# google-research/Splat-SLAM

Measured on AMD Instinct MI355X. Metric: mapping frames/sec + render ms @640x480, 300k Gaussians; PSNR vs ref, higher is better.
Workload: dtype f32

## Files before the change

splat_slam_amd/csrc/sgr_api.hip:

```cpp
#include <cstdarg>
#include <cstdio>
#include <cstring>
#include <cstdlib>
#include <vector>

#include <hip/hip_runtime.h>

#include "sgr_common.h"

namespace sgr {

void launch_preprocess_fwd(const ViewTab&, int, const LOff&, const Common&, const SgrInputs&, hipStream_t);
void launch_preprocess_bwd(const ViewTab&, int, const LOff&, const Common&, const SgrInputs&, const SgrGradInputs&, const FusedAdam*,
                           hipStream_t, bool mapping_loop = false);
void launch_binning(const ViewTab&, int, const LOff&, hipStream_t);
void launch_zero_heads(const ViewTab&, int, const LOff&, size_t, hipStream_t);
void launch_blend_fwd(const ViewTab&, int, const LOff&, const float*, const LossTab*, const LossCoef*, hipStream_t);
void launch_blend_bwd(const ViewTab&, int, const LOff&, const float*, const LossTab*, const LossCoef*, hipStream_t);
void launch_blend_fused(const ViewTab&, int, const LOff&, const float*, const LossTab&, const LossCoef&, hipStream_t);
bool blend_can_fuse(const LOff&);

static int g_opt[SGR_OPT_COUNT] = {1, 0, 0};

static thread_local char g_err[512] = "";
int set_error(int code, const char* fmt, ...) {
  va_list ap;
  va_start(ap, fmt);
  vsnprintf(g_err, sizeof(g_err), fmt, ap);
  va_end(ap);
  return code;
}
#define HIP_TRY(expr)                                                                                   \
  do {                                                                                                  \
    hipError_t _e = (expr);                                                                             \
    if (_e != hipSuccess) return set_error(SGR_ERR_HIP, "%s failed: %s", #expr, hipGetErrorString(_e)); \
  } while (0)
// ... 267 lines not shown
      LOff d = L.dev();
      launch_blend_bwd(tab, 1, d, m.settings.bg, nullptr, nullptr, st);
      launch_preprocess_bwd(tab, 1, d, cm, *in, gv, nullptr, st);
    }
    HIP_TRY(hipGetLastError());
    return SGR_OK;
  }
  Layout L = make_layout(f.settings.num_gaussians, f.settings.image_height, f.settings.image_width, f.ws.capacity);
  LOff d = L.dev();
  Common cm = make_common(&f.settings);
  for (int base = 0; base < num_views; base += kMaxViews) {
    const int nv = num_views - base < kMaxViews ? num_views - base : kMaxViews;
    ViewTab tab = {};
    for (int v = 0; v < nv; ++v) {
      const SgrBackwardView& m = views[base + v];
      if (int rc = check_workspace(&m.ws, L)) return rc;
      tab_set_view(tab, v, &m.settings, nullptr, &m.ws);
      tab.radii[v] = const_cast<int32_t*>(m.radii);
      tab.dL_dcolor[v] = m.dL_dcolor; tab.dL_ddepth[v] = m.dL_ddepth; tab.dL_dtau[v] = m.dL_dtau; tab.dL_dmeans2D[v] = m.dL_dmeans2D;
    }
    SgrGradInputs gv = g;
    gv.accumulate = (grad_in->accumulate || base > 0) ? 1 : 0;
    launch_blend_bwd(tab, nv, d, f.settings.bg, nullptr, nullptr, st);
    launch_preprocess_bwd(tab, nv, d, cm, *in, gv, nullptr, st);
  }
  HIP_TRY(hipGetLastError());
  return SGR_OK;
}

}

static int map_views_impl(int32_t num_views, const SgrMapView* views, const SgrInputs* in, const SgrGradInputs* grads, float alpha,
                          float rgb_boundary_threshold, int32_t forward_only, FusedAdam* fused, bool* fused_done,
                          void* stream, bool store_sinks = false, const SgrSsimTerm* term = nullptr) {
  if (fused_done) *fused_done = false;
  if (num_views < 0 || (num_views > 0 && (!views || !in)) || (!forward_only && !grads))
    return set_error(SGR_ERR_INVALID, "map_views: null argument");
  if (num_views == 0) return SGR_OK;
  if (forward_only) term = nullptr;
  if (term) {
    if (!term->arena || term->max_views <= 0)
      return set_error(SGR_ERR_INVALID, "map_views: SSIM term without an arena");
    for (int v = 0; v < num_views; ++v) {
      const SgrMapView& m = views[v];
      const int H = m.settings.image_height, W = m.settings.image_width;
      if (!m.out.color || !m.out.depth || !m.out.opacity)
        return set_error(SGR_ERR_INVALID, "map_views: the SSIM loss needs every view's rendered image, depth and opacity");
      if (term->arena_bytes < sgr_ssim_term_bytes(term->max_views, H, W))
        return set_error(SGR_ERR_WORKSPACE, "map_views: SSIM arena too small (need %zu for %d views of %dx%d)",
                         sgr_ssim_term_bytes(term->max_views, H, W), term->max_views, W, H);
      if (!m.loss_scratch || m.loss_scratch_bytes < (size_t)ssim_loss_nparts(H, W) * sizeof(LossPart))
        return set_error(SGR_ERR_WORKSPACE, "map_views: loss_scratch too small for the SSIM loss (need %zu)",
                         (size_t)ssim_loss_nparts(H, W) * sizeof(LossPart));
    }
  }
  hipStream_t st = (hipStream_t)stream;
  bool uniform = true;
  const SgrMapView& f = views[0];
  for (int v = 0; v < num_views; ++v) {
    const SgrMapView& m = views[v];
    if (int rc = check_settings(&m.settings, in)) return rc;
    uniform = uniform && m.settings.num_gaussians == f.settings.num_gaussians && m.settings.image_height == f.settings.image_height &&
              m.settings.image_width == f.settings.image_width && m.settings.tanfovx == f.settings.tanfovx &&
              m.settings.tanfovy == f.settings.tanfovy && m.settings.scale_modifier == f.settings.scale_modifier &&
              m.settings.sh_degree == f.settings.sh_degree && m.settings.sh_coeffs == f.settings.sh_coeffs &&
              m.settings.bg == f.settings.bg &&
              m.ws.capacity == f.ws.capacity;
// ... 38 lines not shown
  }
  Layout L = make_layout(f.settings.num_gaussians, f.settings.image_height, f.settings.image_width, f.ws.capacity);
  LOff d = L.dev();
  int hint = 0;
  for (int v = 0; v < num_views; ++v) hint = views[v].ws.max_list_hint > hint ? views[v].ws.max_list_hint : hint;
  d.set_hint(hint);
  Common cm = make_common(&f.settings);
  const int HW = f.settings.image_height * f.settings.image_width;
  for (int base = 0; base < num_views; base += kMaxViews) {
    const int nv = num_views - base < kMaxViews ? num_views - base : kMaxViews;
    ViewTab tab = {};
    LossTab lt = {};
    bool all_clean = true;
    for (int v = 0; v < nv; ++v) {
      const SgrMapView& m = views[base + v];
      all_clean = all_clean && m.ws.counters_clean != 0;
      if (int rc = check_workspace(&m.ws, L)) return rc;
      const bool no_images = !m.out.color && !m.out.depth && !m.out.opacity && !forward_only;
      if ((!no_images && (!m.out.color || !m.out.depth || !m.out.opacity)) || !m.out.radii)
        return set_error(SGR_ERR_INVALID, "map_views: null output pointer");
      tab_set_view(tab, v, &m.settings, &m.out, &m.ws);
      if (!forward_only) {
        if (!m.gt_image || !m.gt_depth || !m.dL_dimage || !m.dL_ddepth || !m.loss_scratch ||
            m.loss_scratch_bytes < (size_t)L.ntiles * sizeof(LossPart))
          return set_error(SGR_ERR_INVALID, "map_views: loss buffers missing (loss_scratch needs 16 B per 8x8 tile = %zu)",
                           (size_t)L.ntiles * sizeof(LossPart));
        tab.dL_dcolor[v] = m.dL_dimage; tab.dL_ddepth[v] = m.dL_ddepth; tab.dL_dtau[v] = m.dL_dtau;
        lt.image[v] = m.out.color; lt.depth[v] = m.out.depth; lt.gt_image[v] = m.gt_image; lt.gt_depth[v] = m.gt_depth;
        lt.exp_a[v] = m.exposure_a; lt.exp_b[v] = m.exposure_b; lt.loss[v] = m.loss; lt.dimage[v] = m.dL_dimage;
        lt.ddepth[v] = m.dL_ddepth; lt.da[v] = m.dL_dexposure; lt.db[v] = m.dL_dexposure ? m.dL_dexposure + 1 : nullptr;
        lt.parts[v] = m.loss_scratch;
      }
    }
    if (int rc = forward_batch(tab, nv, L, cm, *in, st, all_clean, d.mean_hint)) return rc;
    if (forward_only) {
      launch_blend_fwd(tab, nv, d, f.settings.bg, nullptr, nullptr, st);
      continue;
    }
    LossCoef lc = {alpha / (3.f * (float)HW), (1.f - alpha) / (float)HW, rgb_boundary_threshold};
    const bool fused_blend = !term && g_opt[SGR_OPT_FUSED_BLEND] != 0 && blend_can_fuse(d);
    int nparts = L.ntiles;
    if (term) {
      const int H = f.settings.image_height, W = f.settings.image_width;
      launch_blend_fwd(tab, nv, d, f.settings.bg, nullptr, nullptr, st);
      for (int g0 = 0; g0 < nv; g0 += term->max_views)
        launch_ssim_mapping_loss(lt, g0, nv - g0 < term->max_views ? nv - g0 : term->max_views, H, W, alpha, term->lambda_dssim,
                                 rgb_boundary_threshold, 1.f, (float*)term->arena, st);
      nparts = ssim_loss_nparts(H, W);
    } else if (fused_blend) {
      launch_blend_fused(tab, nv, d, f.settings.bg, lt, lc, st);
    } else {
      launch_blend_fwd(tab, nv, d, f.settings.bg, &lt, &lc, st);
    }
    const bool fuse = fused && num_views <= kMaxViews;
    if (fuse) {
      fused->tail_views = nv; fused->tail_nparts = nparts;
      fused->tail_inv_rgb = 1.f / (3.f * (float)HW); fused->tail_inv_dep = 1.f / (float)HW; fused->tail_alpha = alpha;
      for (int v = 0; v < nv; ++v) {
        fused->tail_parts[v] = lt.parts[v]; fused->tail_loss[v] = lt.loss[v]; fused->tail_da[v] = lt.da[v]; fused->tail_db[v] = lt.db[v];
      }
    } else {
      launch_mapping_loss_final(lt, nv, HW, nparts, alpha, st);
    }
    if (term) launch_blend_bwd(tab, nv, d, f.settings.bg, nullptr, nullptr, st);
    else if (!fused_blend) launch_blend_bwd(tab, nv, d, f.settings.bg, &lt, &lc, st);
    launch_preprocess_bwd(tab, nv, d, cm, *in, *grads, fuse ? fused : nullptr, st, true);
    if (fuse && fused_done) *fused_done = true;
  }
  HIP_TRY(hipGetLastError());
  return SGR_OK;
}

extern "C" {

int sgr_map_views(int32_t num_views, const SgrMapView* views, const SgrInputs* in, const SgrGradInputs* grads, float alpha,
                  float rgb_boundary_threshold, int32_t forward_only, void* stream) {
  return map_views_impl(num_views, views, in, grads, alpha, rgb_boundary_threshold, forward_only, nullptr, nullptr, stream);
}

}

static int map_step_impl(const SgrMapStep* p, bool skip_activate, bool grads_clean, bool allow_fuse, bool* fused_out, void* stream,
                         const SgrSsimTerm* term = nullptr) {
  if (fused_out) *fused_out = false;
  if (!p) return set_error(SGR_ERR_INVALID, "map_step: null argument");
  const bool adam_only = p->num_views == 0 && p->adam_groups;
  if (!skip_activate && !adam_only && (p->scaling || p->rotation || p->opacity))
    if (int rc = sgr_activate(p->num_gaussians, p->scaling, p->rotation, p->opacity, p->scales_out, p->rot_out, p->opac_out, stream)) return rc;
  FusedAdam fa;
  bool try_fuse = false;
  if (allow_fuse && p->adam_groups && p->num_views > 0 && p->num_views <= kMaxViews && !p->forward_only && p->grads && p->in && p->views) {
    const SgrGradInputs& g = *p->grads;
    const SgrAdamGroup* G = p->adam_groups;
    try_fuse = g.accumulate && g.dL_dmeans3D == G[0].grad && g.dL_dshs == G[1].grad && g.dL_dopacities == G[2].grad &&
               g.dL_dscales == G[3].grad && g.dL_drotations == G[4].grad && !g.dL_dmeans2D && !g.dL_dcolors_precomp &&
               !g.dL_dcov3D_precomp && p->in->shs && !p->in->colors_precomp && p->in->scales && p->in->rotations &&
               p->num_gaussians == p->views[0].settings.num_gaussians;
    for (int v = 0; v < p->num_views && try_fuse; ++v)
      try_fuse = !p->views[v].dL_dtau && p->views[v].settings.sh_degree == 0 && p->views[v].settings.sh_coeffs == 1;
    if (try_fuse) {
      if (int rc = make_fused_adam(p->num_gaussians, G, p->beta1, p->beta2, p->eps, p->iso_weight, &fa)) return rc;
      fa.grads_clean = grads_clean ? 1 : 0;
      fa.s_out = p->scales_out; fa.r_out = p->rot_out; fa.o_out = p->opac_out;
      fa.stat_accum = g.stat_grad_accum;
      fa.stat_denom = g.stat_grad_accum ? g.stat_denom : nullptr;
      fa.stat_maxr = g.stat_grad_accum ? g.stat_max_radii : nullptr;
      if (p->exp_rows > 0) {
        if (!p->exp_param || !p->exp_grad || !p->exp_avg || !p->exp_avg_sq || !p->exp_step || !p->exp_active || p->exp_row_width <= 0)
          return set_error(SGR_ERR_INVALID, "map_step: exposure block incomplete");
        fa.exp_rows = p->exp_rows; fa.exp_width = p->exp_row_width; fa.exp_param = p->exp_param; fa.exp_grad = p->exp_grad;
        fa.exp_avg = p->exp_avg; fa.exp_avg_sq = p->exp_avg_sq; fa.exp_step = p->exp_step; fa.exp_active = p->exp_active;
        fa.exp_lr = p->exp_lr; fa.exp_b1 = p->exp_beta1; fa.exp_b2 = p->exp_beta2; fa.exp_eps = p->exp_eps;
      }
    }
  }
  if ((p->grads_clean == -2 || p->grads_clean == -3) && !p->adam_groups && p->num_views > 0 && p->num_views <= kMaxViews && !p->forward_only && p->grads &&
      p->in && p->views) {
    const SgrGradInputs& g = *p->grads;
    try_fuse = g.accumulate && g.dL_dmeans3D && g.dL_dshs && g.dL_dopacities && g.dL_dscales && g.dL_drotations &&
               !g.dL_dmeans2D && !g.dL_dcolors_precomp && !g.dL_dcov3D_precomp && p->in->shs && !p->in->colors_precomp &&
               p->in->scales && p->in->rotations && p->num_gaussians == p->views[0].settings.num_gaussians;
    for (int v = 0; v < p->num_views && try_fuse; ++v)
      try_fuse = !p->views[v].dL_dtau && p->views[v].settings.sh_degree == 0 && p->views[v].settings.sh_coeffs == 1;
    if (try_fuse) {
      fa = FusedAdam{};
      fa.gather_only = p->grads_clean == -3 ? 2 : 1;
      fa.G.g[0].grad = g.dL_dmeans3D; fa.G.g[1].grad = g.dL_dshs; fa.G.g[2].grad = g.dL_dopacities;
      fa.G.g[3].grad = g.dL_dscales; fa.G.g[4].grad = g.dL_drotations;
      fa.stat_accum = g.stat_grad_accum;
      fa.stat_denom = g.stat_grad_accum ? g.stat_denom : nullptr;
      fa.stat_maxr = g.stat_grad_accum ? g.stat_max_radii : nullptr;
      if (p->exp_rows > 0) {
        if (!p->exp_param || !p->exp_grad || !p->exp_avg || !p->exp_avg_sq || !p->exp_step || !p->exp_active || p->exp_row_width <= 0)
          return set_error(SGR_ERR_INVALID, "map_step: exposure block incomplete");
        fa.exp_rows = p->exp_rows; fa.exp_width = p->exp_row_width; fa.exp_param = p->exp_param; fa.exp_grad = p->exp_grad;
        fa.exp_avg = p->exp_avg; fa.exp_avg_sq = p->exp_avg_sq; fa.exp_step = p->exp_step; fa.exp_active = p->exp_active;
        fa.exp_lr = p->exp_lr; fa.exp_b1 = p->exp_beta1; fa.exp_b2 = p->exp_beta2; fa.exp_eps = p->exp_eps;
      }
    }
  }
  bool fused = false;
  if (p->num_views > 0)
    if (int rc = map_views_impl(p->num_views, p->views, p->in, p->grads, p->alpha, p->rgb_boundary_threshold, p->forward_only,
                                try_fuse ? &fa : nullptr, &fused, stream, p->grads_clean == -3 && !p->adam_groups, term))
      return rc;
  if (p->adam_groups && !fused)
    if (int rc = gaussian_adam_step_act(p->num_gaussians, p->adam_groups, p->beta1, p->beta2, p->eps, p->iso_weight,
                                        adam_only && p->scaling ? p->scales_out : nullptr,
                                        adam_only && p->rotation ? p->rot_out : nullptr,
                                        adam_only && p->opacity ? p->opac_out : nullptr, stream))
      return rc;
  if (p->exp_rows > 0 && !fused)
    if (int rc = sgr_masked_adam(p->exp_rows, p->exp_row_width, p->exp_param, p->exp_grad, p->exp_avg, p->exp_avg_sq, p->exp_step,
                                 p->exp_active, p->exp_lr, p->exp_beta1, p->exp_beta2, p->exp_eps, stream))
      return rc;
  if (fused_out) *fused_out = fused;
  return SGR_OK;
}

extern "C" {

int sgr_map_step(const SgrMapStep* p, void* stream) {
  if (!p) return set_error(SGR_ERR_INVALID, "map_step: null argument");
  return map_step_impl(p, false, p->grads_clean > 0, p->grads_clean >= 0, nullptr, stream);
}

int sgr_map_step_ssim(const SgrMapStep* p, const SgrSsimTerm* term, void* stream) {
  if (!p) return set_error(SGR_ERR_INVALID, "map_step: null argument");
  return map_step_impl(p, false, p->grads_clean > 0, p->grads_clean >= 0, nullptr, stream, term);
}

}

static int map_run_impl(const SgrMapRun* r, const SgrSsimTerm* term, void* stream) {
  if (!r || r->num_iters < 0 || r->num_window < 0 || r->picks_per_iter < 0 || (r->num_window > 0 && !r->window) ||
      (r->picks_per_iter > 0 && (!r->pool || !r->picks || r->pool_size <= 0)))
    return set_error(SGR_ERR_INVALID, "map_run: bad argument");
  const int nv = r->num_window + r->picks_per_iter;
  if (nv > 64) return set_error(SGR_ERR_INVALID, "map_run: more than 64 views per iteration");
  SgrMapView views[64];
  for (int v = 0; v < r->num_window; ++v) views[v] = r->window[v];
  std::vector<char> pool_used((size_t)(r->pool_size > 0 ? r->pool_size : 0), 0);
  std::vector<char> slot_used((size_t)(r->picks_per_iter > 0 ? r->picks_per_iter : 0), 0);
  SgrMapStep st = r->step;
  st.views = views;
  st.num_views = nv;
  st.adam_groups = r->adam_groups;
  const int32_t exp_rows = st.exp_rows;
  bool prev_fused = false;
  for (int it = 0; it < r->num_iters; ++it) {
    for (int j = 0; j < r->picks_per_iter; ++j) {
      const int32_t k = r->picks[(size_t)it * r->picks_per_iter + j];
      if (k < 0 || k >= r->pool_size) return set_error(SGR_ERR_INVALID, "map_run: pick %d outside the pool", k);
      views[r->num_window + j] = r->pool[k];
      if (r->pick_ws) {
        views[r->num_window + j].ws = r->pick_ws[j];
        if (slot_used[j]) views[r->num_window + j].ws.counters_clean = 1;
        slot_used[j] = 1;
      } else if (pool_used[k]) {
        views[r->num_window + j].ws.counters_clean = 1;
      }
      pool_used[k] = 1;
    }
    if (it == 1)
      for (int v = 0; v < r->num_window; ++v) views[v].ws.counters_clean = 1;
    if (r->n_touched_last_only) {
      const bool last = it == r->num_iters - 1;
      for (int v = 0; v < r->num_window; ++v) views[v].out.n_touched = last ? r->window[v].out.n_touched : nullptr;
      if (!last)
        for (int j = 0; j < r->picks_per_iter; ++j) views[r->num_window + j].out.n_touched = nullptr;
    }
    if (r->adam_groups) {
      if (r->lr0) r->adam_groups[0].lr = r->lr0[it];
      for (int g = 0; g < 5; ++g)
        if (!r->adam_groups[g].skip) r->adam_groups[g].step += 1;
    }
    if (r->pool_exp_row && r->picks_per_iter > 0 && exp_rows > 0) {
      const int32_t row = r->pool_exp_row[r->picks[(size_t)it * r->picks_per_iter]];
      const size_t o = (size_t)(row < 0 ? 0 : row) * (size_t)st.exp_row_width;
      st.exp_rows = row < 0 ? 0 : 1;
      st.exp_param = r->step.exp_param + o; st.exp_grad = r->step.exp_grad + o;
      st.exp_avg = r->step.exp_avg + o; st.exp_avg_sq = r->step.exp_avg_sq + o;
      st.exp_step = r->step.exp_step + (row < 0 ? 0 : row);
    }
    bool fused = false;
    if (int rc = map_step_impl(&st, prev_fused, it == 0 ? r->step.grads_clean > 0 : r->adam_groups != nullptr, r->step.grads_clean >= 0,
                               &fused, stream, term))
      return rc;
    prev_fused = fused;
  }
  return SGR_OK;
}

extern "C" {

int sgr_map_run(const SgrMapRun* r, void* stream) { return map_run_impl(r, nullptr, stream); }
int sgr_map_run_ssim(const SgrMapRun* r, const SgrSsimTerm* term, void* stream) { return map_run_impl(r, term, stream); }

int sgr_query_stats(const SgrWorkspace* ws, int32_t N, int32_t H, int32_t W, const int32_t* radii, int64_t stats_host[4],
                    void* stream) {
  if (!ws || !ws->saved || !ws->scratch || !stats_host) return set_error(SGR_ERR_INVALID, "null argument");
  Layout L = make_layout(N, H, W, ws->capacity);
  hipStream_t st = (hipStream_t)stream;
  unsigned long long* d = (unsigned long long*)ws->scratch;
  HIP_TRY(hipMemsetAsync(d, 0, 32, st));
  hipLaunchKernelGGL(stats_kernel, dim3(64), dim3(256), 0, st, N, L.ntiles, radii, (const uint2*)((char*)ws->saved + L.o_ranges),
                     (const uint32_t*)((char*)ws->saved + L.o_tile_maxc), d);
  unsigned long long h[4];
  HIP_TRY(hipMemcpyAsync(h, d, 32, hipMemcpyDeviceToHost, st));
  HIP_TRY(hipStreamSynchronize(st));
  for (int i = 0; i < 4; ++i) stats_host[i] = (int64_t)h[i];
  return SGR_OK;
}

int sgr_query_depth_keys(const SgrWorkspace* ws, int32_t N, int32_t H, int32_t W, const int32_t* radii, float* depth_out, void* stream) {
  if (!ws || !ws->saved || !radii || !depth_out) return set_error(SGR_ERR_INVALID, "null argument");
  Layout L = make_layout(N, H, W, ws->capacity);
  if (N > 0)
    hipLaunchKernelGGL(depth_keys_kernel, dim3((N + 255) / 256), dim3(256), 0, (hipStream_t)stream, N,
                       (const GRec*)((const char*)ws->saved + L.o_grec), radii, depth_out);
// ... 69 lines not shown
```

splat_slam_amd/csrc/sgr_aux.hip:

```cpp
#include <cmath>

#include <cstdint>

#include "sgr_common.h"

namespace sgr {
int set_error(int code, const char* fmt, ...);


__global__ void __launch_bounds__(256) mapping_loss_kernel(LossTab tab, int HW, float w_rgb, float w_dep, float thr) {
  const int vw = blockIdx.y;
  const float* __restrict__ image = tab.image[vw];
  const float* __restrict__ depth = tab.depth[vw];
  const float* __restrict__ gt_image = tab.gt_image[vw];
  const float* __restrict__ gt_depth = tab.gt_depth[vw];
  float* __restrict__ dimage = tab.dimage[vw];
  float* __restrict__ ddepth = tab.ddepth[vw];
  LossPart* __restrict__ parts = (LossPart*)tab.parts[vw];
  const float ea = tab.exp_a[vw] ? __expf(tab.exp_a[vw][0]) : 1.f;
  const float eb = tab.exp_b[vw] ? tab.exp_b[vw][0] : 0.f;
  LossPart acc = {0.f, 0.f, 0.f, 0.f};
  for (int p = blockIdx.x * blockDim.x + threadIdx.x; p < HW; p += gridDim.x * blockDim.x) {
    float g0 = gt_image[p], g1 = gt_image[HW + p], g2 = gt_image[2 * HW + p];
    bool m = (g0 + g1 + g2) > thr;
// ... 286 lines not shown
      *(float4*)(r_out + 4 * i) = make_float4(pp[0] / nn, pp[1] / nn, pp[2] / nn, pp[3] / nn);
    }
  }
}

__global__ void __launch_bounds__(256) gaussian_adam_kernel(int64_t n, AdamGroups G, AdamConst c, float iso_coef,
                                                            float* __restrict__ s_out, float* __restrict__ r_out,
                                                            float* __restrict__ o_out) {
  int64_t i = (int64_t)blockIdx.x * blockDim.x + threadIdx.x;
  if (i >= n) return;
  const float zero[14] = {0.f, 0.f, 0.f, 0.f, 0.f, 0.f, 0.f, 0.f, 0.f, 0.f, 0.f, 0.f, 0.f, 0.f};
  gaussian_adam_one<0>(i, G, c, iso_coef, zero, s_out, r_out, o_out);
}

template <int MODE>
__global__ void __launch_bounds__(256) gather_adam_kernel(ViewTab tab, int nviews, LOff L, FusedAdam fa) {
  if ((int)blockIdx.x < fa.tail_views) {
    __shared__ LossPart red[4];
    const int v = blockIdx.x;
    loss_final_view((const LossPart*)fa.tail_parts[v], fa.tail_nparts, fa.tail_inv_rgb, fa.tail_inv_dep, fa.tail_alpha,
                    fa.tail_loss[v], fa.tail_da[v], fa.tail_db[v], red);
    if (threadIdx.x == 0 && fa.exp_rows > 0 && fa.tail_da[v] && ((const SavedHeader*)tab.saved[v])->overflow == 0u) {
      const ptrdiff_t d = fa.tail_da[v] - fa.exp_grad;
      if (d >= 0 && d < (ptrdiff_t)fa.exp_rows * fa.exp_width && d % fa.exp_width == 0) {
        const int r = (int)(d / fa.exp_width);
        if (fa.exp_active[r])
          masked_adam_row(r, fa.exp_width, fa.exp_param, fa.exp_grad, fa.exp_avg, fa.exp_avg_sq, fa.exp_step, fa.exp_lr,
                          fa.exp_b1, fa.exp_b2, fa.exp_eps);
      }
    }
    return;
  }
  __shared__ const char* s_scratch[kMaxViews];
  __shared__ const int32_t* s_radii[kMaxViews];
  __shared__ uint32_t s_over[kMaxViews];
#pragma unroll
  for (int u = 0; u < kMaxViews; ++u)
    if ((int)threadIdx.x == u && u < nviews) {
      s_scratch[u] = tab.scratch[u];
      s_radii[u] = tab.radii[u];
      s_over[u] = ((const SavedHeader*)tab.saved[u])->overflow;
    }
  __syncthreads();
  uint32_t truncated = 0u;
  for (int u = 0; u < nviews; ++u) truncated |= (s_over[u] != 0u ? 1u : 0u) << u;
  const int i = ((int)blockIdx.x - fa.tail_views) * blockDim.x + threadIdx.x;
  if (i >= L.N) return;
  float a[14];
#pragma unroll
  for (int k = 0; k < 14; ++k) a[k] = 0.f;
  float st_norm = 0.f, st_cnt = 0.f, st_maxr = 0.f;
  uint32_t seen = 0u;
  for (int p = 0; p < min(L.k1_parts, nviews); ++p) seen |= ((const uint32_t*)(tab.saved[0] + L.o_vismask))[(size_t)p * L.N + i];
  seen &= ~truncated;
  const bool any = seen != 0u;
  while (seen) {
    const int v = __builtin_ctz(seen);
    seen &= seen - 1u;
    const float4* rec = (const float4*)(s_scratch[v] + L.o_gradrec) + (size_t)i * 4;
    const int r = s_radii[v][i];
    float4 r0 = rec[0], r1 = rec[1], r2 = rec[2], r3 = rec[3];
    a[0] += r0.x; a[1] += r0.y; a[2] += r0.z; a[3] += r0.w; a[4] += r1.x; a[5] += r1.y; a[6] += r1.z; a[7] += r1.w;
    a[8] += r2.x; a[9] += r2.y; a[10] += r2.z; a[11] += r2.w; a[12] += r3.x; a[13] += r3.y;
    st_norm += sqrtf(r3.z * r3.z + r3.w * r3.w);
    st_cnt += 1.f;
    st_maxr = fmaxf(st_maxr, (float)r);
  }
  if (any && fa.stat_accum) {
    fa.stat_accum[i] += st_norm;
    fa.stat_denom[i] += st_cnt;
    fa.stat_maxr[i] = fmaxf(fa.stat_maxr[i], st_maxr);
  }
  if (MODE == 3) {
    if (!any) return;
    float* g0 = fa.G.g[0].grad + 3 * (size_t)i; float* g1 = fa.G.g[1].grad + 3 * (size_t)i; float* g3 = fa.G.g[3].grad + 3 * (size_t)i;
    float* g4 = fa.G.g[4].grad + 4 * (size_t)i;
    g0[0] += a[0]; g0[1] += a[1]; g0[2] += a[2];
    g1[0] += a[3]; g1[1] += a[4]; g1[2] += a[5];
    fa.G.g[2].grad[i] += a[6];
    g3[0] += a[7]; g3[1] += a[8]; g3[2] += a[9];
    g4[0] += a[10]; g4[1] += a[11]; g4[2] += a[12]; g4[3] += a[13];
    return;
  }
  if (MODE == 4) {
    st3(fa.G.g[0].grad + 3 * (size_t)i, F3{a[0], a[1], a[2]});
    st3(fa.G.g[1].grad + 3 * (size_t)i, F3{a[3], a[4], a[5]});
    fa.G.g[2].grad[i] = a[6];
    st3(fa.G.g[3].grad + 3 * (size_t)i, F3{a[7], a[8], a[9]});
    *(float4*)(fa.G.g[4].grad + 4 * (size_t)i) = make_float4(a[10], a[11], a[12], a[13]);
    return;
  }
  gaussian_adam_one<MODE >= 3 ? 1 : MODE>(i, fa.G, fa.c, fa.iso_coef, a, fa.s_out, fa.r_out, fa.o_out);
}
// ... 529 lines not shown
```

splat_slam_amd/csrc/sgr_common.h:

```cpp
#pragma once

#include <hip/hip_runtime.h>
#include <stdint.h>

#include "../../include/splat_hip.h"

namespace sgr {

constexpr float kNearPlane = 0.001f;
constexpr float kAlphaMin = 1.0f / 255.0f;
constexpr float kAlphaMax = 0.99f;
constexpr float kTEps = 1e-4f;
constexpr float kDilation = 0.3f;
constexpr float kTouchedT = 0.5f;
constexpr int kRefTile = 16;
constexpr int kTile = 8;
constexpr int kWave = 64;
constexpr int kCntSlotWords = 8;
constexpr uint32_t kTileCountLimit = 0xff00u;
__host__ __device__ inline size_t tile_counter_word(int x, int y, int gxp) { return ((size_t)(y >> 1) * gxp + (x >> 1)) * (kCntSlotWords / 2); }
__host__ __device__ inline int tile_counter_shift(int x, int y) { return 16 * ((y & 1) * 2 + (x & 1)); }
constexpr int kK1MaxParts = 4;
#ifndef SGR_K1_DENSE_PARTS
#define SGR_K1_DENSE_PARTS 2
// ... 96 lines not shown
  float* dL_dmeans2D[kMaxViews];
};
struct LOff {
  int N, H, W, gx, gy, gxp, sgx, sgy, ntiles, pre_blocks, nseg, dbg, mean_hint, k1_parts;
  uint32_t sgx_magic;
  __host__ void set_hint(int h) { mean_hint = h; k1_parts = k1_parts_for(nseg, h); }
  int64_t cap;
  size_t o_hdr, o_tile_count, o_grec, o_point_list, o_ranges,
      o_tile_maxc, o_final_T, o_tile_order, o_block_touched, o_block_vis, o_block_base_t, o_block_base_v, o_vis_list,
      o_seg_list, o_vismask, o_entries, o_bucket, o_ovf, o_partials, o_tau_part, o_gradrec, o_taurec;
};
#ifndef SGR_TILE_ORDER_MIN_LIST
#define SGR_TILE_ORDER_MIN_LIST 64
#endif
__host__ __device__ inline bool tile_order_used(const LOff& L) { return !(L.mean_hint != 0 && L.mean_hint <= SGR_TILE_ORDER_MIN_LIST); }
struct __attribute__((aligned(16))) OvfEntry { uint32_t tile, rank; uint64_t key; };
struct Common {
  int deg, M;
  int upstream_pose_jac;
  float tanfovx, tanfovy, mod;
  const float* bg;
};

int debug_flags();

struct __attribute__((aligned(16))) GRec {
  float px, py;
  uint32_t rect01, rect23;
  float A, B, C, opacity;
  float r, g, b, depth;
  uint32_t touched, offset, vis_pos, clamped;
};
static_assert(sizeof(GRec) == 64, "GRec must be one 64-byte record");
struct Rect { int x0, y0, x1, y1; };
__device__ __forceinline__ Rect unpack_rect(uint32_t r01, uint32_t r23) {
  return {(int)(r01 & 0xffffu), (int)(r01 >> 16), (int)(r23 & 0xffffu), (int)(r23 >> 16)};
}

struct Layout {
  int N, H, W;
  int64_t cap;
  int gx, gy, ntiles;
  int sgx, sgy;
  int tile_bits;
  size_t o_hdr, o_tile_count, o_grec, o_point_list, o_ranges,
      o_tile_maxc, o_final_T, o_tile_order, o_block_touched, o_block_vis, o_block_base_t, o_block_base_v, o_vis_list,
      o_seg_list, o_vismask, saved_bytes, zero_bytes;
  size_t o_entries, o_bucket, o_ovf;
  size_t o_partials, o_tau_part, o_gradrec, o_taurec, scratch_bytes;
  int pre_blocks, nseg;

  __host__ Layout(int N_, int H_, int W_, int64_t cap_) : N(N_), H(H_), W(W_), cap(cap_) {
    gx = (W + kTile - 1) / kTile;
    gy = (H + kTile - 1) / kTile;
    ntiles = gx * gy;
    sgx = (W + kRefTile - 1) / kRefTile;
    sgy = (H + kRefTile - 1) / kRefTile;
    tile_bits = 1;
    while ((1ll << tile_bits) < (long long)ntiles + 1) ++tile_bits;
    size_t o = 0;
    auto take = [&](size_t bytes) { size_t r = o; o = align_up(o + bytes); return r; };
    size_t n = (size_t)(N > 0 ? N : 1), c = (size_t)(cap > 0 ? cap : 1);
    pre_blocks = (N + 255) / 256;
    nseg = (N + kSeg - 1) / kSeg;
    size_t nb = (size_t)(pre_blocks > 0 ? pre_blocks : 1);
    o_hdr = take(sizeof(SavedHeader));
// ... 181 lines not shown
```

splat_slam_amd/csrc/sgr_preprocess.hip:

```cpp
#include "sgr_common.h"

namespace sgr {

struct Cam {
  float vm[16];
  float pm[16];
};

__device__ __forceinline__ void load16(const float* __restrict__ src, float* dst) {
#pragma unroll
  for (int i = 0; i < 16; ++i) dst[i] = src[i];
}

__device__ __forceinline__ void quat_to_R(const float q[4], float R[3][3]) {
  float r = q[0], x = q[1], y = q[2], z = q[3];
  R[0][0] = 1.f - 2.f * (y * y + z * z); R[0][1] = 2.f * (x * y - r * z); R[0][2] = 2.f * (x * z + r * y);
  R[1][0] = 2.f * (x * y + r * z); R[1][1] = 1.f - 2.f * (x * x + z * z); R[1][2] = 2.f * (y * z - r * x);
  R[2][0] = 2.f * (x * z - r * y); R[2][1] = 2.f * (y * z + r * x); R[2][2] = 1.f - 2.f * (x * x + y * y);
}

__device__ __forceinline__ void cov3d_from_scale_rot(const float s[3], float mod, const float q[4], float S6[6]) {
  float R[3][3];
  quat_to_R(q, R);
  float M[3][3];
// ... 342 lines not shown
            const float pad = 1e-3f * (fabsf(a) + fabsf(bsum)) + 1e-4f;
            v0[r] = a - pad; v1[r] = bsum + pad;
          }
          if (v1[2] <= kNearPlane) {
            maybe = false;
          } else if (v0[2] > kNearPlane) {
            const float fx = L.W / (2.f * cm.tanfovx), fy = L.H / (2.f * cm.tanfovy);
            const float iz0 = 1.f / v0[2], iz1 = 1.f / v1[2];
            const float xz0 = fminf(fminf(v0[0] * iz0, v0[0] * iz1), fminf(v1[0] * iz0, v1[0] * iz1));
            const float xz1 = fmaxf(fmaxf(v0[0] * iz0, v0[0] * iz1), fmaxf(v1[0] * iz0, v1[0] * iz1));
            const float yz0 = fminf(fminf(v0[1] * iz0, v0[1] * iz1), fminf(v1[1] * iz0, v1[1] * iz1));
            const float yz1 = fmaxf(fmaxf(v0[1] * iz0, v0[1] * iz1), fmaxf(v1[1] * iz0, v1[1] * iz1));
            const float limx = 1.3f * cm.tanfovx, limy = 1.3f * cm.tanfovy;
            const float tn = (fx * fx * (1.f + limx * limx) + fy * fy * (1.f + limy * limy)) * iz0 * iz0;
            const float rad = ceilf(3.f * sqrtf(tn * tsm * 1.01f + 1.0f)) + 3.f;
            const float ox = 0.5f * L.W * (p_projraw[tid][8] + 1.f) - 0.5f, oy = 0.5f * L.H * (p_projraw[tid][9] + 1.f) - 0.5f;
            const float px0 = fx * xz0 + ox - rad - 1.f, px1 = fx * xz1 + ox + rad + (kRefTile - 1) + 1.f;
            const float py0 = fy * yz0 + oy - rad - 1.f, py1 = fy * yz1 + oy + rad + (kRefTile - 1) + 1.f;
            if (isfinite(px0) && isfinite(px1) && isfinite(py0) && isfinite(py1) && isfinite(rad))
              maybe = !(px1 < 0.f || py1 < 0.f || px0 >= (float)(L.sgx * kRefTile) || py0 >= (float)(L.sgy * kRefTile));
          }
        }
        if (maybe) atomicOr(&seg_views, 1u << tid);
      }
      __syncthreads();
    }
    const uint32_t segv = seg_views;
    const float sroot = __builtin_amdgcn_sqrtf(fmaxf(trS, 0.f)) * 1.0005f;
#pragma unroll 2
    for (int v = 0; v < nviews; ++v) {
      bool pass = false;
      if (ia < N && (v % nparts) == part) {
        if (!(L.dbg & 16)) {
        p_radii[v][ia] = 0;
        if (p_ntouched[v]) p_ntouched[v][ia] = 0;
        }
        if (L.dbg & 2) pass = (p[0] + trS == 12345.678f);
        else if (segv & (1u << v)) pass = (L.dbg & 8) ? maybe_visible(p, trS, L.H, L.W, cm.tanfovx, cm.tanfovy, mats[v], mats[v] + 16, L.sgx, L.sgy)
                                                      : maybe_visible_planes(p, sroot, mats[v], mats[v] + 16, cullK[v], L.H, L.W, L.sgx, L.sgy);
      }
      const unsigned long long m = __ballot(pass);
      if (lane == 0) wtot[v][wv] = (uint32_t)__popcll(m);
      if (pass) {
        passbits |= 1u << v;
        ranks[v >> 2] |= (uint32_t)__popcll(m & ((1ull << lane) - 1ull)) << ((v & 3) * 8);
      }
    }
  }
  __syncthreads();
  if (tid == 0) {
    uint32_t run = 0;
    for (int v = 0; v < nviews; ++v) {
      vstart[v] = run;
      run += wtot[v][0] + wtot[v][1] + wtot[v][2] + wtot[v][3];
    }
    for (int v = nviews; v <= kMaxViews; ++v) vstart[v] = run;
  }
#pragma unroll 1
  for (int v = 0; v < nviews; ++v) {
    if (passbits & (1u << v)) {
      const uint32_t base = (wv > 0 ? wtot[v][0] : 0u) + (wv > 1 ? wtot[v][1] : 0u) + (wv > 2 ? wtot[v][2] : 0u);
      cand[v][base + ((ranks[v >> 2] >> ((v & 3) * 8)) & 0xffu)] = (uint8_t)tid;
    }
  }
  __syncthreads();
  const uint32_t total = (L.dbg & 1) ? 0u : vstart[kMaxViews];

  uint32_t carry_t = 0, carry_v = 0;
#pragma unroll 1
  for (uint32_t f0 = 0; f0 < total; f0 += 256) {
    const uint32_t f = f0 + tid;
    const bool live = f < total;
    int v = 0;
#pragma unroll
    for (int u = 1; u < kMaxViews; ++u) v += (f >= vstart[u] && u < nviews) ? 1 : 0;
    PreOut o;
    o.visible = false;
    o.x0 = o.x1 = o.y0 = o.y1 = 0;
    int i = 0;
    char* saved = p_saved[v];
    if (live) {
      i = seg0 + (int)cand[v][f - vstart[v]];
      const float* vm = mats[v];
      const float* pm = mats[v] + 16;
      PreIn in;
      { const F3 t = ld3(means3D + 3 * i); in.p[0] = t.x; in.p[1] = t.y; in.p[2] = t.z; }
      in.opac = opacities[i];
      if (cov3D_precomp) {
#pragma unroll
        for (int k = 0; k < 6; ++k) in.S6[k] = cov3D_precomp[6 * i + k];
      } else {
        const F3 sc3 = ld3(scales + 3 * i);
        const float4 q4 = *(const float4*)(rotations + 4 * i);
        float s_in[3] = {sc3.x, sc3.y, sc3.z};
        float q_in[4] = {q4.x, q4.y, q4.z, q4.w};
        cov3d_from_scale_rot(s_in, cm.mod, q_in, in.S6);
      }
      in.c_in[0] = in.c_in[1] = in.c_in[2] = 0.f;
      if (colors_precomp) { in.c_in[0] = colors_precomp[3 * i]; in.c_in[1] = colors_precomp[3 * i + 1]; in.c_in[2] = colors_precomp[3 * i + 2]; }
      else if (cm.deg == 0) { in.c_in[0] = shs[(size_t)i * cm.M * 3]; in.c_in[1] = shs[(size_t)i * cm.M * 3 + 1]; in.c_in[2] = shs[(size_t)i * cm.M * 3 + 2]; }
      preprocess_view(in, i, L.H, L.W, cm.deg, cm.M, cm.tanfovx, cm.tanfovy, vm, pm, p_campos[v], shs,
                      colors_precomp != nullptr, L.gx, L.gy, L.sgx, L.sgy, o);
    }
    const uint32_t cnt = o.visible ? (uint32_t)((o.x1 - o.x0) * (o.y1 - o.y0)) : 0u;
    const uint32_t vis = o.visible ? 1u : 0u;
    if (o.visible && !(L.dbg & 128)) {
      atomicOr(&vis_bits[i - seg0], 1u << v);
      p_radii[v][i] = (int32_t)o.rad;
      float4* rec = (float4*)((GRec*)(saved + L.o_grec) + i);
      rec[0] = make_float4(o.px, o.py, __uint_as_float((uint32_t)o.x0 | ((uint32_t)o.y0 << 16)),
                           __uint_as_float((uint32_t)o.x1 | ((uint32_t)o.y1 << 16)));
      rec[1] = make_float4(o.A, o.B, o.C, o.opac);
      rec[2] = make_float4(o.rgb[0], o.rgb[1], o.rgb[2], o.depth);
    }
    const uint32_t my_rx = (uint32_t)o.x0 | ((uint32_t)o.x1 << 16), my_ry = (uint32_t)o.y0 | ((uint32_t)o.y1 << 16);
    const uint32_t nops = cnt > 0u ? (uint32_t)((((o.x1 - 1) >> 1) - (o.x0 >> 1) + 1) * (((o.y1 - 1) >> 1) - (o.y0 >> 1) + 1)) : 0u;
    op_rect[tid] = make_uint4(my_rx, my_ry, (uint32_t)v, (uint32_t)i);
    op_depth[tid] = __float_as_uint(o.depth);
    Footprint my_foot{0.f, 0.f, 0.f, 0.f, 0.f, 0.f, 0.f, -1.f};
    if (o.visible && footprint_worthwhile(o.x1 - o.x0, o.y1 - o.y0)) my_foot = make_footprint(o.px, o.py, o.A, o.B, o.C, o.opac, 0.005f);
    op_foot[tid][0] = make_float4(my_foot.px, my_foot.py, my_foot.A, my_foot.B);
    op_foot[tid][1] = make_float4(my_foot.C, my_foot.invA, my_foot.invC, my_foot.thr);
    auto op_geom = [](uint32_t rx, uint32_t ry, int k, const Footprint& foot) -> uint32_t {
      const int x0 = (int)(rx & 0xffffu), x1 = (int)(rx >> 16), y0 = (int)(ry & 0xffffu), y1 = (int)(ry >> 16);
      const int per_row = ((x1 - 1) >> 1) - (x0 >> 1) + 1;
      int q = (int)(((float)k + 0.5f) * __builtin_amdgcn_rcpf((float)per_row));
      int rem = k - q * per_row;
      if (rem < 0) { --q; rem += per_row; }
      if (rem >= per_row) { ++q; rem -= per_row; }
      const int bx = ((x0 >> 1) + rem) * 2, by = ((y0 >> 1) + q) * 2;
      const bool c0 = bx >= x0, c1 = bx + 1 < x1, r0 = by >= y0, r1 = by + 1 < y1;
      uint32_t cover = (uint32_t)(r0 && c0) | ((uint32_t)(r0 && c1) << 1) | ((uint32_t)(r1 && c0) << 2) | ((uint32_t)(r1 && c1) << 3);
      if (foot.thr >= 0.f) {
        const float drop = foot.thr * kFootDrop + kFootGuard;
#pragma unroll
        for (int s4 = 0; s4 < 4; ++s4)
          if (((cover >> s4) & 1u) && footprint_qmin(foot, bx + (s4 & 1), by + (s4 >> 1)) > drop) cover &= ~(1u << s4);
      }
      return (uint32_t)bx | ((uint32_t)by << 14) | (cover << 28);
    };
    auto issue = [&](int view, uint32_t geo) -> unsigned long long {
      const uint32_t cover = geo >> 28;
      if (cover == 0u || (L.dbg & 32)) return 0ull;
      const unsigned long long inc = (unsigned long long)(cover & 1u) | ((unsigned long long)((cover >> 1) & 1u) << 16) |
                                     ((unsigned long long)((cover >> 2) & 1u) << 32) | ((unsigned long long)((cover >> 3) & 1u) << 48);
      unsigned long long* c = (unsigned long long*)(p_saved[view] + L.o_tile_count) +
                              tile_counter_word((int)(geo & 0x3fffu), (int)((geo >> 14) & 0x3fffu), L.gxp);
      return atomicAdd(c, (L.dbg & 64) ? 0ull : inc);
    };
    struct Desc { int view; uint64_t key; };
    auto desc_of = [&](int owner) -> Desc {
      const uint2 vz = *(const uint2*)&op_rect[owner].z;
      return Desc{(int)vz.x, ((uint64_t)op_depth[owner] << 32) | vz.y};
// ... 70 lines not shown
    auto issue_round = [&](uint32_t it0, uint32_t tot_r) {
#pragma unroll
      for (int jj = 0; jj < 4; ++jj) {
        const uint32_t item = it0 + (uint32_t)jj * 256u + (uint32_t)tid;
        owner4[jj] = -1;
        if (item < tot_r) {
          int lo = 0, hi = 256;
          while (lo < hi) { const int mid = (lo + hi) >> 1; if (op_ex[mid] <= item) lo = mid + 1; else hi = mid; }
          owner4[jj] = lo - 1;
          const uint4 r = op_rect[lo - 1];
          const float4 f0 = op_foot[lo - 1][0], f1 = op_foot[lo - 1][1];
          geo4[jj] = op_geom(r.x, r.y, 4 + (int)(item - op_ex[lo - 1]), Footprint{f0.x, f0.y, f0.z, f0.w, f1.x, f1.y, f1.z, f1.w});
          old4[jj] = issue((int)r.z, geo4[jj]);
        }
      }
    };
    auto consume_round = [&]() { consume4(old4, geo4, owner4); };
#pragma unroll
    for (int jj = 0; jj < 4; ++jj) {
      owner4[jj] = jj < (int)nops ? tid : -1;
      if (jj < (int)nops) { geo4[jj] = op_geom(my_rx, my_ry, jj, my_foot); old4[jj] = issue(v, geo4[jj]); }
    }
    uint32_t tot_t, tot_v;
    const uint32_t ex_t = carry_t + block256_exclusive_scan(cnt, red, tot_t);
    const uint32_t ex_v = carry_v + block256_exclusive_scan(vis, red, tot_v);
    if (live) {
#pragma unroll
      for (int u = 1; u <= kMaxViews; ++u)
        if (u > v && vstart[u] == f + 1) { vbase_t[u] = ex_t + cnt; vbase_v[u] = ex_v + vis; }
    }
    __syncthreads();
    if (o.visible) {
      const uint32_t k = ex_v - vbase_v[v];
      ((uint4*)((GRec*)(saved + L.o_grec) + i))[3] = make_uint4(cnt, ex_t - vbase_t[v], k, o.clamped);
      ((uint32_t*)(saved + L.o_seg_list))[seg0 + k] = (uint32_t)i;
    }
    consume_round();
    const uint32_t rem = nops > 4u ? nops - 4u : 0u;
    if (__syncthreads_or(rem > 0u)) {
      uint32_t tot_r;
      op_ex[tid] = block256_exclusive_scan(rem, red, tot_r);
      __syncthreads();
#pragma unroll 1
      for (uint32_t it0 = 0; it0 < tot_r; it0 += 4u * 256u) {
        issue_round(it0, tot_r);
        consume_round();
      }
    }
    __syncthreads();
    carry_t += tot_t;
    carry_v += tot_v;
  }
  __syncthreads();
  if (ia < N) ((uint32_t*)(p_saved[0] + L.o_vismask))[(size_t)part * N + ia] = vis_bits[tid];
  if (tid < nviews && (tid % nparts) == part) {
    char* saved = p_saved[tid];
    ((uint32_t*)(saved + L.o_block_touched))[seg] = vbase_t[tid + 1] - vbase_t[tid];
    ((uint32_t*)(saved + L.o_block_vis))[seg] = vbase_v[tid + 1] - vbase_v[tid];
  }
}

struct GaussGrad {
  float p[3], s[3], q[4], S6[6], op, m2[2], rgb_or_sh0[3];
};

__device__ __forceinline__ void preprocess_bwd_one_view(
    int i, int H, int W, int deg, int M, float tanfovx, float tanfovy, float mod, const float* __restrict__ viewmatrix,
// ... 351 lines not shown
        }
#pragma unroll
        for (int off = 1; off < 64; off <<= 1)
#pragma unroll
          for (int j = 0; j < 10; ++j) part[j] += __shfl_xor(part[j], off);
        if ((lane & ~(LPG - 1)) == src)
#pragma unroll
          for (int j = 0; j < 10; ++j) gsum[j] = part[j];
      }
    }
  }
  if (!have || (LPG > 1 && (threadIdx.x & (LPG - 1)) != 0)) return;
  {
    const float G0 = gsum[0], G1 = gsum[1], Gxx = gsum[2], Gxy = gsum[3], Go = gsum[4], Gr = gsum[5], Gg = gsum[6], Gb = gsum[7],
                Gyy = gsum[8], Gd = gsum[9];
    gsum[0] = (-(g1.x * G0) - g1.y * G1) * (0.5f * (float)L.W);
    gsum[1] = (-(g1.z * G1) - g1.y * G0) * (0.5f * (float)L.H);
    gsum[2] = -0.5f * Gxx;
    gsum[3] = -Gxy;
    gsum[4] = -0.5f * Gyy;
    gsum[5] = Go; gsum[6] = Gr; gsum[7] = Gg; gsum[8] = Gb; gsum[9] = Gd;
  }
  float tau[6] = {0.f, 0.f, 0.f, 0.f, 0.f, 0.f};
  GaussGrad acc;
#pragma unroll
  for (int j = 0; j < 3; ++j) { acc.p[j] = 0.f; acc.s[j] = 0.f; acc.rgb_or_sh0[j] = 0.f; }
#pragma unroll
  for (int j = 0; j < 4; ++j) acc.q[j] = 0.f;
#pragma unroll
  for (int j = 0; j < 6; ++j) acc.S6[j] = 0.f;
  acc.op = 0.f; acc.m2[0] = 0.f; acc.m2[1] = 0.f;
  preprocess_bwd_one_view(i, L.H, L.W, cm.deg, cm.M, cm.tanfovx, cm.tanfovy, cm.mod, tab.viewmatrix[v], tab.projmatrix[v],
                          tab.projraw[v], tab.campos[v], means3D, shs, colors_precomp, scales, rotations, cov3D_precomp,
                          gsum, q3.w, dshs, accumulate, acc, tau, cm.upstream_pose_jac);
  float4* rec = (float4*)(tab.scratch[v] + L.o_gradrec) + (size_t)i * 4;
  rec[0] = make_float4(acc.p[0], acc.p[1], acc.p[2], acc.rgb_or_sh0[0]);
  rec[1] = make_float4(acc.rgb_or_sh0[1], acc.rgb_or_sh0[2], acc.op, acc.s[0]);
  rec[2] = make_float4(acc.s[1], acc.s[2], acc.q[0], acc.q[1]);
  rec[3] = make_float4(acc.q[2], acc.q[3], acc.m2[0], acc.m2[1]);
  if (float* m2 = tab.dL_dmeans2D[v]) {
    if (((const SavedHeader*)(saved + L.o_hdr))->overflow == 0u) {
      m2[3 * (size_t)i] = acc.m2[0];
      m2[3 * (size_t)i + 1] = acc.m2[1];
    }
  }
  if (dcov3D) {
#pragma unroll
    for (int j = 0; j < 6; ++j) { if (accumulate) dcov3D[6 * i + j] += acc.S6[j]; else dcov3D[6 * i + j] = acc.S6[j]; }
  }
  if (tab.dL_dtau[v]) {
    float* tr = (float*)(tab.scratch[v] + L.o_taurec) + (size_t)t * 6;
#pragma unroll
    for (int j = 0; j < 6; ++j) tr[j] = tau[j];
  }
}

__global__ void __launch_bounds__(256) grad_gather_kernel(
    ViewTab tab, int nviews, LOff L, int deg, int M, int has_colors, float* __restrict__ dmeans3D,
    float* __restrict__ dmeans2D, float* __restrict__ dopac, float* __restrict__ dshs, float* __restrict__ dcolors,
    float* __restrict__ dscales, float* __restrict__ drots, float* __restrict__ dcov3D, int accumulate,
    float* __restrict__ stat_accum, float* __restrict__ stat_denom, float* __restrict__ stat_maxr) {
  __shared__ float red[4][6];
  const int i = blockIdx.x * blockDim.x + threadIdx.x;
  const bool in_range = i < L.N;
  float a[14];
#pragma unroll
  for (int k = 0; k < 14; ++k) a[k] = 0.f;
// ... 123 lines not shown
```

Measured before the change: 63.19.

## Pack radius into GRec clamp word and skip dead radii writes

Packs each Gaussian's screen radius into the upper bits of the GRec clamped word, so the Adam/accumulate kernel reads the radius from the saved record instead of a separate radii array. The host computes, for each mapping-loop iteration, which views' radii outputs will be overwritten later and nulls those pointers so preprocess skips the global radii stores. The first three GRec float4 writes are moved after the scan and rebuilt from shared-memory op state, coalescing them with the fourth record write. This cuts redundant global traffic but adds a host-side hash map pass and relies on the low 3 bits carrying clamp flags.

```diff
diff --git a/splat_slam_amd/csrc/sgr_api.hip b/splat_slam_amd/csrc/sgr_api.hip
--- a/splat_slam_amd/csrc/sgr_api.hip
+++ b/splat_slam_amd/csrc/sgr_api.hip
@@ -2,6 +2,7 @@
 #include <cstdio>
 #include <cstring>
 #include <cstdlib>
+#include <unordered_map>
 #include <vector>
 
 #include <hip/hip_runtime.h>
@@ -335,7 +336,7 @@
 
 static int map_views_impl(int32_t num_views, const SgrMapView* views, const SgrInputs* in, const SgrGradInputs* grads, float alpha,
                           float rgb_boundary_threshold, int32_t forward_only, FusedAdam* fused, bool* fused_done,
-                          void* stream, bool store_sinks = false, const SgrSsimTerm* term = nullptr) {
+                          void* stream, bool store_sinks = false, const SgrSsimTerm* term = nullptr, uint64_t radii_dead = 0) {
   if (fused_done) *fused_done = false;
   if (num_views < 0 || (num_views > 0 && (!views || !in)) || (!forward_only && !grads))
     return set_error(SGR_ERR_INVALID, "map_views: null argument");
@@ -440,6 +441,9 @@
         lt.parts[v] = m.loss_scratch;
       }
     }
+    if (!forward_only && fused && num_views <= kMaxViews)
+      for (int v = 0; v < nv; ++v)
+        if ((radii_dead >> v) & 1u) tab.radii[v] = nullptr;
     if (int rc = forward_batch(tab, nv, L, cm, *in, st, all_clean, d.mean_hint)) return rc;
     if (forward_only) {
       launch_blend_fwd(tab, nv, d, f.settings.bg, nullptr, nullptr, st);
@@ -489,7 +493,7 @@
 }
 
 static int map_step_impl(const SgrMapStep* p, bool skip_activate, bool grads_clean, bool allow_fuse, bool* fused_out, void* stream,
-                         const SgrSsimTerm* term = nullptr) {
+                         const SgrSsimTerm* term = nullptr, uint64_t radii_dead = 0) {
   if (fused_out) *fused_out = false;
   if (!p) return set_error(SGR_ERR_INVALID, "map_step: null argument");
   const bool adam_only = p->num_views == 0 && p->adam_groups;
@@ -550,7 +554,7 @@
   bool fused = false;
   if (p->num_views > 0)
     if (int rc = map_views_impl(p->num_views, p->views, p->in, p->grads, p->alpha, p->rgb_boundary_threshold, p->forward_only,
-                                try_fuse ? &fa : nullptr, &fused, stream, p->grads_clean == -3 && !p->adam_groups, term))
+                                try_fuse ? &fa : nullptr, &fused, stream, p->grads_clean == -3 && !p->adam_groups, term, radii_dead))
       return rc;
   if (p->adam_groups && !fused)
     if (int rc = gaussian_adam_step_act(p->num_gaussians, p->adam_groups, p->beta1, p->beta2, p->eps, p->iso_weight,
@@ -590,6 +594,13 @@
   for (int v = 0; v < r->num_window; ++v) views[v] = r->window[v];
   std::vector<char> pool_used((size_t)(r->pool_size > 0 ? r->pool_size : 0), 0);
   std::vector<char> slot_used((size_t)(r->picks_per_iter > 0 ? r->picks_per_iter : 0), 0);
+  std::unordered_map<const int32_t*, int> last_render;
+  for (int it = 0; it < r->num_iters; ++it)
+    for (int j = 0; j < r->picks_per_iter; ++j) {
+      const int32_t k = r->picks[(size_t)it * r->picks_per_iter + j];
+      if (k >= 0 && k < r->pool_size) last_render[r->pool[k].out.radii] = it;
+    }
+  for (int v = 0; v < r->num_window; ++v) last_render[r->window[v].out.radii] = r->num_iters - 1;
   SgrMapStep st = r->step;
   st.views = views;
   st.num_views = nv;
@@ -631,9 +642,12 @@
       st.exp_avg = r->step.exp_avg + o; st.exp_avg_sq = r->step.exp_avg_sq + o;
       st.exp_step = r->step.exp_step + (row < 0 ? 0 : row);
     }
+    uint64_t radii_dead = 0;
+    for (int v = 0; v < nv; ++v)
+      if (last_render[views[v].out.radii] != it) radii_dead |= 1ull << v;
     bool fused = false;
     if (int rc = map_step_impl(&st, prev_fused, it == 0 ? r->step.grads_clean > 0 : r->adam_groups != nullptr, r->step.grads_clean >= 0,
-                               &fused, stream, term))
+                               &fused, stream, term, radii_dead))
       return rc;
     prev_fused = fused;
   }
diff --git a/splat_slam_amd/csrc/sgr_aux.hip b/splat_slam_amd/csrc/sgr_aux.hip
--- a/splat_slam_amd/csrc/sgr_aux.hip
+++ b/splat_slam_amd/csrc/sgr_aux.hip
@@ -342,13 +342,13 @@
     return;
   }
   __shared__ const char* s_scratch[kMaxViews];
-  __shared__ const int32_t* s_radii[kMaxViews];
+  __shared__ const char* s_saved[kMaxViews];
   __shared__ uint32_t s_over[kMaxViews];
 #pragma unroll
   for (int u = 0; u < kMaxViews; ++u)
     if ((int)threadIdx.x == u && u < nviews) {
       s_scratch[u] = tab.scratch[u];
-      s_radii[u] = tab.radii[u];
+      s_saved[u] = tab.saved[u];
       s_over[u] = ((const SavedHeader*)tab.saved[u])->overflow;
     }
   __syncthreads();
@@ -368,7 +368,7 @@
     const int v = __builtin_ctz(seen);
     seen &= seen - 1u;
     const float4* rec = (const float4*)(s_scratch[v] + L.o_gradrec) + (size_t)i * 4;
-    const int r = s_radii[v][i];
+    const int r = grec_radius(grec_of(s_saved[v], L)[i].clamped);
     float4 r0 = rec[0], r1 = rec[1], r2 = rec[2], r3 = rec[3];
     a[0] += r0.x; a[1] += r0.y; a[2] += r0.z; a[3] += r0.w; a[4] += r1.x; a[5] += r1.y; a[6] += r1.z; a[7] += r1.w;
     a[8] += r2.x; a[9] += r2.y; a[10] += r2.z; a[11] += r2.w; a[12] += r3.x; a[13] += r3.y;
diff --git a/splat_slam_amd/csrc/sgr_common.h b/splat_slam_amd/csrc/sgr_common.h
--- a/splat_slam_amd/csrc/sgr_common.h
+++ b/splat_slam_amd/csrc/sgr_common.h
@@ -152,6 +152,9 @@
   uint32_t touched, offset, vis_pos, clamped;
 };
 static_assert(sizeof(GRec) == 64, "GRec must be one 64-byte record");
+constexpr uint32_t kGrecClampMask = 7u;
+__device__ __forceinline__ uint32_t grec_pack_radius(int32_t r) { return min((uint32_t)max(r, 0), 0x1fffffffu) << 3; }
+__device__ __forceinline__ int32_t grec_radius(uint32_t word15) { return (int32_t)(word15 >> 3); }
 struct Rect { int x0, y0, x1, y1; };
 __device__ __forceinline__ Rect unpack_rect(uint32_t r01, uint32_t r23) {
   return {(int)(r01 & 0xffffu), (int)(r01 >> 16), (int)(r23 & 0xffffu), (int)(r23 >> 16)};
diff --git a/splat_slam_amd/csrc/sgr_preprocess.hip b/splat_slam_amd/csrc/sgr_preprocess.hip
--- a/splat_slam_amd/csrc/sgr_preprocess.hip
+++ b/splat_slam_amd/csrc/sgr_preprocess.hip
@@ -398,7 +398,7 @@
       bool pass = false;
       if (ia < N && (v % nparts) == part) {
         if (!(L.dbg & 16)) {
-        p_radii[v][ia] = 0;
+        if (p_radii[v]) p_radii[v][ia] = 0;
         if (p_ntouched[v]) p_ntouched[v][ia] = 0;
         }
         if (L.dbg & 2) pass = (p[0] + trS == 12345.678f);
@@ -444,7 +444,6 @@
     o.visible = false;
     o.x0 = o.x1 = o.y0 = o.y1 = 0;
     int i = 0;
-    char* saved = p_saved[v];
     if (live) {
       i = seg0 + (int)cand[v][f - vstart[v]];
       const float* vm = mats[v];
@@ -472,19 +471,18 @@
     const uint32_t vis = o.visible ? 1u : 0u;
     if (o.visible && !(L.dbg & 128)) {
       atomicOr(&vis_bits[i - seg0], 1u << v);
-      p_radii[v][i] = (int32_t)o.rad;
-      float4* rec = (float4*)((GRec*)(saved + L.o_grec) + i);
-      rec[0] = make_float4(o.px, o.py, __uint_as_float((uint32_t)o.x0 | ((uint32_t)o.y0 << 16)),
-                           __uint_as_float((uint32_t)o.x1 | ((uint32_t)o.y1 << 16)));
-      rec[1] = make_float4(o.A, o.B, o.C, o.opac);
-      rec[2] = make_float4(o.rgb[0], o.rgb[1], o.rgb[2], o.depth);
+      if (p_radii[v]) p_radii[v][i] = (int32_t)o.rad;
+      o.clamped |= grec_pack_radius((int32_t)o.rad);
     }
     const uint32_t my_rx = (uint32_t)o.x0 | ((uint32_t)o.x1 << 16), my_ry = (uint32_t)o.y0 | ((uint32_t)o.y1 << 16);
     const uint32_t nops = cnt > 0u ? (uint32_t)((((o.x1 - 1) >> 1) - (o.x0 >> 1) + 1) * (((o.y1 - 1) >> 1) - (o.y0 >> 1) + 1)) : 0u;
     op_rect[tid] = make_uint4(my_rx, my_ry, (uint32_t)v, (uint32_t)i);
     op_depth[tid] = __float_as_uint(o.depth);
     Footprint my_foot{0.f, 0.f, 0.f, 0.f, 0.f, 0.f, 0.f, -1.f};
-    if (o.visible && footprint_worthwhile(o.x1 - o.x0, o.y1 - o.y0)) my_foot = make_footprint(o.px, o.py, o.A, o.B, o.C, o.opac, 0.005f);
+    if (o.visible) {
+      if (footprint_worthwhile(o.x1 - o.x0, o.y1 - o.y0)) my_foot = make_footprint(o.px, o.py, o.A, o.B, o.C, o.opac, 0.005f);
+      else { my_foot.px = o.px; my_foot.py = o.py; my_foot.A = o.A; my_foot.B = o.B; my_foot.C = o.C; }
+    }
     op_foot[tid][0] = make_float4(my_foot.px, my_foot.py, my_foot.A, my_foot.B);
     op_foot[tid][1] = make_float4(my_foot.C, my_foot.invA, my_foot.invC, my_foot.thr);
     auto op_geom = [](uint32_t rx, uint32_t ry, int k, const Footprint& foot) -> uint32_t {
@@ -621,7 +619,16 @@
     __syncthreads();
     if (o.visible) {
       const uint32_t k = ex_v - vbase_v[v];
-      ((uint4*)((GRec*)(saved + L.o_grec) + i))[3] = make_uint4(cnt, ex_t - vbase_t[v], k, o.clamped);
+      char* saved = p_saved[v];
+      const uint4 rc = op_rect[tid];
+      float4* rec = (float4*)((GRec*)(saved + L.o_grec) + rc.w);
+      if (!(L.dbg & 128)) {
+        const float4 f0 = op_foot[tid][0];
+        rec[0] = make_float4(f0.x, f0.y, __uint_as_float((rc.x & 0xffffu) | (rc.y << 16)), __uint_as_float((rc.x >> 16) | (rc.y & 0xffff0000u)));
+        rec[1] = make_float4(f0.z, f0.w, op_foot[tid][1].x, o.opac);
+        rec[2] = make_float4(o.rgb[0], o.rgb[1], o.rgb[2], __uint_as_float(op_depth[tid]));
+      }
+      ((uint4*)rec)[3] = make_uint4(cnt, ex_t - vbase_t[v], k, o.clamped);
       ((uint32_t*)(saved + L.o_seg_list))[seg0 + k] = (uint32_t)i;
     }
     consume_round();
@@ -1039,7 +1046,7 @@
   acc.op = 0.f; acc.m2[0] = 0.f; acc.m2[1] = 0.f;
   preprocess_bwd_one_view(i, L.H, L.W, cm.deg, cm.M, cm.tanfovx, cm.tanfovy, cm.mod, tab.viewmatrix[v], tab.projmatrix[v],
                           tab.projraw[v], tab.campos[v], means3D, shs, colors_precomp, scales, rotations, cov3D_precomp,
-                          gsum, q3.w, dshs, accumulate, acc, tau, cm.upstream_pose_jac);
+                          gsum, q3.w & kGrecClampMask, dshs, accumulate, acc, tau, cm.upstream_pose_jac);
   float4* rec = (float4*)(tab.scratch[v] + L.o_gradrec) + (size_t)i * 4;
   rec[0] = make_float4(acc.p[0], acc.p[1], acc.p[2], acc.rgb_or_sh0[0]);
   rec[1] = make_float4(acc.rgb_or_sh0[1], acc.rgb_or_sh0[2], acc.op, acc.s[0]);
```

New measurement: 62.64. No clear change (-0.9%).
